# chaitjo/efficient-gnns

Hardware: NVIDIA H100
Metric: edges aggregated/s (fwd+bwd), 3-layer GCN student + logit-KD, ARXIV-shape (higher is better)
Workload: dtype f32

## Files before the change

### efficient-gnns_b200/csrc/gemm_tf32x3.cu

```cuda
#include <cuda.h>

#include "common.cuh"
#include "tc_common.cuh"

namespace b200gnn {
namespace gemm {
using namespace tc;

constexpr int BM = 128, BK = 32;
constexpr int THREADS = 384;
constexpr int CONSUMER_WARPS = 8;
constexpr int TILE_BYTES = BM * BK * 4;
constexpr int BAR_BYTES = 256;
constexpr int EPI_BYTES = CONSUMER_WARPS * 16 * 32 * 4;
constexpr int STAT_MAX_N = 256;
constexpr int STAT_BYTES = CONSUMER_WARPS * 2 * STAT_MAX_N * 4;
constexpr int XY_ROWS = 16;
constexpr int XY_SLOT_BYTES = 2 * XY_ROWS * 32 * 4;
constexpr int XY_BYTES = CONSUMER_WARPS * 2 * XY_SLOT_BYTES;
constexpr int XY_BAR_OFF = 128;
constexpr int BNBWD_TMA_MAX_K = 128;

template <int BN_T, int NSTAGE, int EXTRA = 0>
struct Cfg {
  static constexpr int BN = BN_T, STAGES = NSTAGE;
  static constexpr int B_TILE_BYTES = BN_T * BK * 4;
  static constexpr int STAGE_BYTES = TILE_BYTES + 2 * B_TILE_BYTES;
  static constexpr int ACC = BN_T / 2;
  static constexpr int SMEM_BYTES = NSTAGE * STAGE_BYTES + BAR_BYTES + EPI_BYTES + STAT_BYTES + EXTRA + 1024;
  static_assert(B_TILE_BYTES % 1024 == 0 && (BN_T == 128 || BN_T == 48), "tile shape (wgmma wrappers: N = 128, 48)");
  static_assert(2 * NSTAGE * 8 <= XY_BAR_OFF, "barrier block");
  static_assert(SMEM_BYTES <= 232448, "shared memory");
};

__device__ __forceinline__ void mma(float (&d)[64], const uint32_t (&a)[4], uint64_t b, uint32_t s) { wgmma_tf32_n128_rs(d, a, b, s); }
__device__ __forceinline__ void mma(float (&d)[24], const uint32_t (&a)[4], uint64_t b, uint32_t s) { wgmma_tf32_n48_rs(d, a, b, s); }

__device__ __forceinline__ uint32_t a_frag_offset(int r0, int lane) { return r0 * 128 + ((lane >> 2) << 4) + (lane & 3) * 4; }
__device__ __forceinline__ void load_a(uint32_t frag, uint32_t (&v)[BK / 8][4]) {
  asm("" : "+r"(frag));
#pragma unroll
  for (int k = 0; k < BK / 8; ++k)
#pragma unroll
    for (int i = 0; i < 4; ++i) v[k][i] = lds32((frag ^ ((2 * k + (i >> 1)) << 4)) + (i & 1) * 8 * 128);
}

__device__ __forceinline__ int stg(int r, int c4) { return r * 32 + ((c4 ^ (r & 7)) << 2); }

struct Params {
  float* C;
  const float* bias;
  int64_t ldc;
  int32_t M, N, K;
  int32_t accumulate;
  float* Cp[16];
  int32_t n_peer, kc;
  int64_t row_off;
  int32_t bcast;
  int32_t stat_mode;
  float* stat_partial;
  const float* bn_x;
  const float* bn_y;
  const float* bn_mean;
  const float* bn_invstd;
  float inv_keep;
  const float* act_scale;
  const float* act_shift;
  const uint32_t* act_bits;
  int32_t act_words;
  const float* act_slope;
  double* slope_partial;
  const int64_t* row_idx;
};

template <bool ACT>
__device__ __forceinline__ void load_bn_chunk(const Params& p, int m0, int col, int q, int lane, float4 (&x)[4], float4 (&y)[4]) {
  if (col + 32 > p.N) return;
  const int sub = lane >> 3, cq = (lane & 7) * 4;
#pragma unroll
  for (int it = 0; it < 4; ++it) {
    const int grow = m0 + q * 16 + it * 4 + sub;
    if (grow < p.M) {
      const size_t o = (size_t)grow * p.ldc + col + cq;
      if (!ACT) x[it] = __ldg(reinterpret_cast<const float4*>(p.bn_x + o));
      y[it] = __ldg(reinterpret_cast<const float4*>(p.bn_y + o));
    }
  }
}

__device__ __forceinline__ void load_bits_chunk(const Params& p, int m0, int col, int q, int lane, uint32_t (&w)[4]) {
  const int sub = lane >> 3;
#pragma unroll
  for (int it = 0; it < 4; ++it) {
    const int grow = m0 + q * 16 + it * 4 + sub;
    w[it] = grow < p.M ? __ldg(p.act_bits + (size_t)grow * p.act_words + (col >> 5)) : 0u;
  }
}

__device__ __forceinline__ uint32_t act1(uint32_t y, float sc, float sh, uint32_t keep, float inv_keep) {
  return keep ? __float_as_uint(fmaxf(fmaf(__uint_as_float(y), sc, sh), 0.f) * inv_keep) : 0u;
}

__device__ __forceinline__ uint32_t prelu1(uint32_t z, float slope, uint32_t keep, float inv_keep) {
  const float x = __uint_as_float(z);
  return keep ? __float_as_uint((x > 0.f ? x : slope * x) * inv_keep) : 0u;
}

template <class C, int STAT, bool PEER, bool ACT = false, bool PRELU = false, bool ROWIDX = false>
__global__ void __launch_bounds__(THREADS, 1)
gemm_tf32x3_kernel(const __grid_constant__ CUtensorMap tmA, const __grid_constant__ CUtensorMap tmBhi,
                   const __grid_constant__ CUtensorMap tmBlo, const __grid_constant__ CUtensorMap tmX,
                   const __grid_constant__ CUtensorMap tmY, const Params p) {
  constexpr bool BNB = STAT == 2 || STAT == 3;
  constexpr bool XYTMA = STAT == 3;
  constexpr bool COLSTAT = STAT >= 1 && STAT <= 3;
  constexpr bool PRB = STAT == 4;
  constexpr bool PRO = (ACT || PRELU) && !STAT;
  constexpr int BN = C::BN, STAGES = C::STAGES, STAGE_BYTES = C::STAGE_BYTES, B_TILE_BYTES = C::B_TILE_BYTES, ACC = C::ACC;
  extern __shared__ uint8_t smem_raw[];
  uint8_t* smem = reinterpret_cast<uint8_t*>((reinterpret_cast<uintptr_t>(smem_raw) + 1023) & ~(uintptr_t)1023);
  uint64_t* bars = reinterpret_cast<uint64_t*>(smem + STAGES * STAGE_BYTES);
  uint64_t* full = bars;
  uint64_t* empty = bars + STAGES;
  float* epi_smem = reinterpret_cast<float*>(smem + STAGES * STAGE_BYTES + BAR_BYTES);
  float* stat_smem = reinterpret_cast<float*>(smem + STAGES * STAGE_BYTES + BAR_BYTES + EPI_BYTES);
  uint8_t* xy_smem = smem + STAGES * STAGE_BYTES + BAR_BYTES + EPI_BYTES + STAT_BYTES;
  uint64_t* xy_full = reinterpret_cast<uint64_t*>(smem + STAGES * STAGE_BYTES + XY_BAR_OFF);

  const int warp = threadIdx.x >> 5, lane = threadIdx.x & 31;

  if (threadIdx.x == 0) {
    for (int s = 0; s < STAGES; ++s) { mbar_init(&full[s], 1); mbar_init(&empty[s], 256); }
    if (XYTMA)
      for (int i = 0; i < 2 * CONSUMER_WARPS; ++i) mbar_init(&xy_full[i], 1);
    asm volatile("fence.mbarrier_init.release.cluster;" ::: "memory");
  }
  __syncthreads();

  const int num_m = (p.M + BM - 1) / BM, num_n = (p.N + BN - 1) / BN;
  const int num_tiles = num_m * num_n;
  const int num_kb = (p.K + BK - 1) / BK;

  if (warp < 4) {
    regs_dec<40>();
    if (threadIdx.x == 0) {
      int s = 0; uint32_t ph = 0;
      for (int tile = blockIdx.x; tile < num_tiles; tile += gridDim.x) {
        const int m0 = (tile / num_n) * BM, n0 = (tile % num_n) * BN;
        for (int kb = 0; kb < num_kb; ++kb) {
          mbar_wait(&empty[s], ph ^ 1);
          uint8_t* st = smem + s * STAGE_BYTES;
          mbar_expect_tx(&full[s], TILE_BYTES + 2 * B_TILE_BYTES);
          tma_load_2d(&tmA, &full[s], st, kb * BK, m0);
          tma_load_2d(&tmBhi, &full[s], st + TILE_BYTES, kb * BK, n0);
          tma_load_2d(&tmBlo, &full[s], st + TILE_BYTES + B_TILE_BYTES, kb * BK, n0);
          if (++s == STAGES) { s = 0; ph ^= 1; }
        }
      }
    }
    return;
  }
  regs_inc<232>();

  const int q = warp - 4;
  const bool vec_ok = PEER ? true : ((p.ldc % 4 == 0) && ((reinterpret_cast<uintptr_t>(p.C) & 15) == 0));
  float* stat = stat_smem + q * (2 * STAT_MAX_N);
  if (COLSTAT) {
    for (int i = lane; i < 2 * p.N; i += 32) stat[i] = 0.f;
    __syncwarp();
  }
  constexpr int NCHUNK = (BN + 31) / 32;
  uint8_t* xy = xy_smem + q * (2 * XY_SLOT_BYTES);
  uint64_t* xyb = xy_full + q * 2;
  int n_mine = 0;
  if (XYTMA) {
    for (int tt = blockIdx.x; tt < num_tiles; tt += gridDim.x) n_mine += NCHUNK;
    if (lane == 0)
      for (int g = 0; g < 2 && g < n_mine; ++g) {
        const int tt = blockIdx.x + (g / NCHUNK) * gridDim.x, cc = g % NCHUNK;
        mbar_expect_tx(&xyb[g], ACT ? XY_SLOT_BYTES / 2 : XY_SLOT_BYTES);
        if (!ACT)
          tma_load_2d(&tmX, &xyb[g], xy + g * XY_SLOT_BYTES, (tt % num_n) * BN + cc * 32, (tt / num_n) * BM + q * XY_ROWS);
        tma_load_2d(&tmY, &xyb[g], xy + g * XY_SLOT_BYTES + XY_SLOT_BYTES / 2, (tt % num_n) * BN + cc * 32,
                    (tt / num_n) * BM + q * XY_ROWS);
      }
  }
  const float* act_ss = stat_smem;
  if (ACT && !STAT) {
    for (int c = threadIdx.x - 128; c < num_kb * BK; c += 256) {
      const int w = c & 31;
      const float2 v = c < p.K ? make_float2(__ldg(p.act_scale + c), __ldg(p.act_shift + c)) : make_float2(0.f, 0.f);
      *reinterpret_cast<float2*>(stat_smem + (c >> 5) * 64 + (w & 3) * 16 + (w >> 3) * 4 + ((w >> 2) & 1) * 2) = v;
    }
    named_sync(1, 256);
  }
  const int arow = q * 16 + (lane >> 2);
  auto act_words = [&](int tile, int kb, uint32_t (&w)[2]) {
    const int r = (tile / num_n) * BM + arow;
    w[0] = r < p.M ? __ldg(p.act_bits + (size_t)r * p.act_words + kb) : 0u;
    w[1] = r + 8 < p.M ? __ldg(p.act_bits + (size_t)(r + 8) * p.act_words + kb) : 0u;
  };
  uint32_t wnext[2] = {0u, 0u};
  if (PRO && blockIdx.x < num_tiles) act_words(blockIdx.x, 0, wnext);
  const float slope = (PRELU || PRB) ? __ldg(p.act_slope) : 0.f;
  double sg = 0.0;
  float acc[ACC], sum[ACC];
  uint32_t ah0[BK / 8][4], al0[BK / 8][4], ah1[BK / 8][4], al1[BK / 8][4];
  const uint32_t frag = a_frag_offset(q * 16 + (lane >> 2), lane);
  int s = 0; uint32_t ph = 0;
  int g_chunk = 0;
  for (int tile = blockIdx.x; tile < num_tiles; tile += gridDim.x) {
    const int m0 = (tile / num_n) * BM, n0 = (tile % num_n) * BN;
#pragma unroll
    for (int i = 0; i < ACC; ++i) sum[i] = acc[i] = 0.f;
    int prev = 0;
    auto stage = [&](int kb, uint32_t (&h)[BK / 8][4], uint32_t (&l)[BK / 8][4]) {
      uint32_t wcur[2];
      if (PRO) {
        wcur[0] = wnext[0] >> (lane & 3); wcur[1] = wnext[1] >> (lane & 3);
        if (kb + 1 < num_kb) act_words(tile, kb + 1, wnext);
        else if (tile + (int)gridDim.x < num_tiles) act_words(tile + gridDim.x, 0, wnext);
      }
      mbar_wait(&full[s], ph);
      uint8_t* st = smem + s * STAGE_BYTES;
      load_a(smem_u32(st) + frag, h);
      if (ACT && !STAT) {
        const float4* ss = reinterpret_cast<const float4*>(act_ss + kb * 64 + (lane & 3) * 16);
#pragma unroll
        for (int k = 0; k < BK / 8; ++k) {
          const float4 t = ss[k];
#pragma unroll
          for (int i = 0; i < 4; ++i)
            h[k][i] = act1(h[k][i], (i >> 1) ? t.z : t.x, (i >> 1) ? t.w : t.y, (wcur[i & 1] >> (8 * k + 4 * (i >> 1))) & 1u,
                           p.inv_keep);
        }
      }
      if (PRELU && !STAT) {
#pragma unroll
        for (int k = 0; k < BK / 8; ++k)
#pragma unroll
          for (int i = 0; i < 4; ++i)
            h[k][i] = prelu1(h[k][i], slope, (wcur[i & 1] >> (8 * k + 4 * (i >> 1))) & 1u, p.inv_keep);
      }
#pragma unroll
      for (int k = 0; k < BK / 8; ++k)
#pragma unroll
        for (int i = 0; i < 4; ++i) split1(h[k][i], h[k][i], l[k][i]);
      reg_fence(h); reg_fence(l);
      if (kb > 0) {
        wgmma_wait<0>();
        acc_fence(acc);
#pragma unroll
        for (int i = 0; i < ACC; ++i) sum[i] += acc[i];
        mbar_arrive(&empty[prev]);
      }
      wgmma_fence();
      const uint32_t sb = smem_u32(st + TILE_BYTES);
#pragma unroll
      for (int k = 0; k < BK / 8; ++k) {
        const uint32_t koff = k * 32;
        mma(acc, l[k], make_desc_k128(sb + koff), k != 0);
        mma(acc, h[k], make_desc_k128(sb + B_TILE_BYTES + koff), 1);
      }
#pragma unroll
      for (int k = 0; k < BK / 8; ++k) mma(acc, h[k], make_desc_k128(sb + k * 32), 1);
      wgmma_commit();
      prev = s;
      if (++s == STAGES) { s = 0; ph ^= 1; }
    };
    for (int kb = 0; kb < num_kb; kb += 2) {
      stage(kb, ah0, al0);
      if (kb + 1 < num_kb) stage(kb + 1, ah1, al1);
    }
    wgmma_wait<0>();
    acc_fence(acc);
#pragma unroll
    for (int i = 0; i < ACC; ++i) sum[i] += acc[i];
    mbar_arrive(&empty[prev]);

    float* tile_s = epi_smem + q * (16 * 32);
#pragma unroll
    for (int c = 0; c < NCHUNK; ++c, ++g_chunk) {
      const int col0 = n0 + c * 32;
      float4 xr[4], yr[4];
      if (STAT == 2) load_bn_chunk<ACT>(p, m0, col0, q, lane, xr, yr);
      if (PRB) load_bn_chunk<true>(p, m0, col0, q, lane, xr, yr);
#pragma unroll
      for (int jj = 0; jj < 4; ++jj) {
        const int j = c * 4 + jj;
        if (j * 8 < BN) {
          const int r0 = lane >> 2, cc = jj * 8 + 2 * (lane & 3);
          *reinterpret_cast<float2*>(tile_s + stg(r0, cc >> 2) + (cc & 3)) = make_float2(sum[4 * j], sum[4 * j + 1]);
          *reinterpret_cast<float2*>(tile_s + stg(r0 + 8, cc >> 2) + (cc & 3)) = make_float2(sum[4 * j + 2], sum[4 * j + 3]);
        }
      }
      __syncwarp();
      if (vec_ok && col0 + 32 <= p.N) {
        const float* xs = reinterpret_cast<const float*>(xy + (g_chunk & 1) * XY_SLOT_BYTES);
        const float* ys = xs + XY_ROWS * 32;
        if (XYTMA) mbar_wait(&xyb[g_chunk & 1], (uint32_t)((g_chunk >> 1) & 1));
        const int sub = lane >> 3, cq = (lane & 7) * 4;
        float4 b4 = make_float4(0.f, 0.f, 0.f, 0.f);
        if (p.bias) b4 = make_float4(__ldg(p.bias + col0 + cq), __ldg(p.bias + col0 + cq + 1), __ldg(p.bias + col0 + cq + 2),
                                     __ldg(p.bias + col0 + cq + 3));
        float4 s4 = make_float4(0.f, 0.f, 0.f, 0.f), q4 = s4, mu4 = s4, is4 = s4, sc4 = s4, sh4 = s4;
        if (BNB) {
          mu4 = __ldg(reinterpret_cast<const float4*>(p.bn_mean + col0 + cq));
          is4 = __ldg(reinterpret_cast<const float4*>(p.bn_invstd + col0 + cq));
        }
        uint32_t wb[4];
        if (BNB && ACT) {
          sc4 = __ldg(reinterpret_cast<const float4*>(p.act_scale + col0 + cq));
          sh4 = __ldg(reinterpret_cast<const float4*>(p.act_shift + col0 + cq));
          load_bits_chunk(p, m0, col0, q, lane, wb);
        }
        if (PRB) load_bits_chunk(p, m0, col0, q, lane, wb);
#pragma unroll
        for (int it = 0; it < 4; ++it) {
          const int rr = it * 4 + sub;
          const int grow = m0 + q * 16 + rr;
          float4 v = *reinterpret_cast<const float4*>(tile_s + stg(rr, lane & 7));
          v.x += b4.x; v.y += b4.y; v.z += b4.z; v.w += b4.w;
          if (PEER && grow < p.M && p.bcast) {
            for (int r = 0; r < p.n_peer; ++r)
              *reinterpret_cast<float4*>(p.Cp[r] + (size_t)(p.row_off + grow) * p.ldc + col0 + cq) = v;
          } else if (grow < p.M) {
            float4* dst;
            if (PEER) {
              const int r = col0 / p.kc;
              dst = reinterpret_cast<float4*>(p.Cp[r] + (size_t)(p.row_off + grow) * p.kc + (col0 - r * p.kc) + cq);
            } else {
              const int64_t crow = ROWIDX ? __ldg(p.row_idx + grow) : (int64_t)grow;
              dst = reinterpret_cast<float4*>(p.C + (size_t)crow * p.ldc + col0 + cq);
            }
            if (!PEER && p.accumulate) { const float4 o = *dst; v.x += o.x; v.y += o.y; v.z += o.z; v.w += o.w; }
            if (STAT == 1) {
              vstat(s4, q4, v);
            } else if (BNB) {
              float4 x = make_float4(0.f, 0.f, 0.f, 0.f);
              if (!ACT) x = XYTMA ? *reinterpret_cast<const float4*>(xs + rr * 32 + cq) : xr[it];
              const float4 y = XYTMA ? *reinterpret_cast<const float4*>(ys + rr * 32 + cq) : yr[it];
              if (ACT) {
                const uint32_t b = wb[it] >> cq;
                v.x = (b & 1u) && fmaf(y.x, sc4.x, sh4.x) > 0.f ? v.x * p.inv_keep : 0.f;
                v.y = (b & 2u) && fmaf(y.y, sc4.y, sh4.y) > 0.f ? v.y * p.inv_keep : 0.f;
                v.z = (b & 4u) && fmaf(y.z, sc4.z, sh4.z) > 0.f ? v.z * p.inv_keep : 0.f;
                v.w = (b & 8u) && fmaf(y.w, sc4.w, sh4.w) > 0.f ? v.w * p.inv_keep : 0.f;
              } else {
                v.x = x.x > 0.f ? v.x * p.inv_keep : 0.f; v.y = x.y > 0.f ? v.y * p.inv_keep : 0.f;
                v.z = x.z > 0.f ? v.z * p.inv_keep : 0.f; v.w = x.w > 0.f ? v.w * p.inv_keep : 0.f;
              }
              s4.x += v.x; s4.y += v.y; s4.z += v.z; s4.w += v.w;
              q4.x = fmaf(v.x, (y.x - mu4.x) * is4.x, q4.x); q4.y = fmaf(v.y, (y.y - mu4.y) * is4.y, q4.y);
              q4.z = fmaf(v.z, (y.z - mu4.z) * is4.z, q4.z); q4.w = fmaf(v.w, (y.w - mu4.w) * is4.w, q4.w);
            } else if (PRB) {
              const float4 z = yr[it];
              const uint32_t b = wb[it] >> cq;
              const float gx = (b & 1u) ? v.x * p.inv_keep : 0.f, gy = (b & 2u) ? v.y * p.inv_keep : 0.f;
              const float gz = (b & 4u) ? v.z * p.inv_keep : 0.f, gw = (b & 8u) ? v.w * p.inv_keep : 0.f;
              if (!(z.x > 0.f)) sg += (double)(gx * z.x);
              if (!(z.y > 0.f)) sg += (double)(gy * z.y);
              if (!(z.z > 0.f)) sg += (double)(gz * z.z);
              if (!(z.w > 0.f)) sg += (double)(gw * z.w);
              v.x = z.x > 0.f ? gx : gx * slope; v.y = z.y > 0.f ? gy : gy * slope;
              v.z = z.z > 0.f ? gz : gz * slope; v.w = z.w > 0.f ? gw : gw * slope;
            }
            *dst = v;
          }
        }
        if (COLSTAT) {
#pragma unroll
          for (int d = 8; d <= 16; d <<= 1) {
            s4.x += __shfl_xor_sync(0xffffffffu, s4.x, d); s4.y += __shfl_xor_sync(0xffffffffu, s4.y, d);
            s4.z += __shfl_xor_sync(0xffffffffu, s4.z, d); s4.w += __shfl_xor_sync(0xffffffffu, s4.w, d);
            q4.x += __shfl_xor_sync(0xffffffffu, q4.x, d); q4.y += __shfl_xor_sync(0xffffffffu, q4.y, d);
            q4.z += __shfl_xor_sync(0xffffffffu, q4.z, d); q4.w += __shfl_xor_sync(0xffffffffu, q4.w, d);
          }
          if (lane < 8) {
            float4* ps = reinterpret_cast<float4*>(stat + col0 + cq);
            float4* pq = reinterpret_cast<float4*>(stat + p.N + col0 + cq);
            float4 a0 = *ps, a1 = *pq;
            a0.x += s4.x; a0.y += s4.y; a0.z += s4.z; a0.w += s4.w;
            a1.x += q4.x; a1.y += q4.y; a1.z += q4.z; a1.w += q4.w;
            *ps = a0; *pq = a1;
          }
        }
        __syncwarp();
        if (XYTMA && lane == 0 && g_chunk + 2 < n_mine) {
          const int g = g_chunk + 2, tt = blockIdx.x + (g / NCHUNK) * gridDim.x, cc = g % NCHUNK;
          uint8_t* dst = xy + (g & 1) * XY_SLOT_BYTES;
          mbar_expect_tx(&xyb[g & 1], ACT ? XY_SLOT_BYTES / 2 : XY_SLOT_BYTES);
          if (!ACT) tma_load_2d(&tmX, &xyb[g & 1], dst, (tt % num_n) * BN + cc * 32, (tt / num_n) * BM + q * XY_ROWS);
          tma_load_2d(&tmY, &xyb[g & 1], dst + XY_SLOT_BYTES / 2, (tt % num_n) * BN + cc * 32, (tt / num_n) * BM + q * XY_ROWS);
        }
      } else {
        const int rr = lane & 15, cb = (lane >> 4) * 16, grow = m0 + q * 16 + rr;
        if (grow < p.M && col0 + cb < p.N) {
          for (int jx = 0; jx < 16; ++jx) {
            const int cc = cb + jx, col = col0 + cc;
            if (col >= p.N) break;
            const float v = tile_s[stg(rr, cc >> 2) + (cc & 3)] + (p.bias ? __ldg(p.bias + col) : 0.f);
            if (PEER && p.bcast) {
              for (int r = 0; r < p.n_peer; ++r) p.Cp[r][(size_t)(p.row_off + grow) * p.ldc + col] = v;
            } else if (!PEER) {
              float* dst = p.C + (size_t)(ROWIDX ? __ldg(p.row_idx + grow) : (int64_t)grow) * p.ldc + col;
              *dst = v + (p.accumulate ? *dst : 0.f);
            }
          }
        }
        __syncwarp();
      }
    }
  }
  if (COLSTAT) {
    __syncwarp();
    float* out = p.stat_partial + (size_t)(blockIdx.x * CONSUMER_WARPS + q) * 2 * p.N;
    for (int i = lane; i < 2 * p.N; i += 32) out[i] = stat[i];
  }
  if (PRB) {
#pragma unroll
    for (int d = 16; d > 0; d >>= 1) sg += __shfl_xor_sync(0xffffffffu, sg, d);
    if (lane == 0) p.slope_partial[blockIdx.x * CONSUMER_WARPS + q] = sg;
  }
}

__global__ void __launch_bounds__(32) slope_grad_finalize_kernel(const double* __restrict__ part, int n, float* __restrict__ out,
                                                                 int accumulate) {
  double a = 0.0;
  for (int i = threadIdx.x; i < n; i += 32) a += part[i];
#pragma unroll
  for (int d = 16; d > 0; d >>= 1) a += __shfl_xor_sync(0xffffffffu, a, d);
  if (threadIdx.x == 0) out[0] = accumulate ? out[0] + (float)a : (float)a;
}

__global__ void __launch_bounds__(256) split_tf32_kernel(const float* __restrict__ W, int64_t rows, int64_t cols,
                                                         int transpose, float* __restrict__ hi, float* __restrict__ lo) {
  const int64_t n = rows * cols;
  for (int64_t i = (int64_t)blockIdx.x * blockDim.x + threadIdx.x; i < n; i += (int64_t)gridDim.x * blockDim.x) {
    const int64_t r = i / cols, c = i - r * cols;
    uint32_t h, l;
    split1(__float_as_uint(W[i]), h, l);
    const int64_t o = transpose ? c * rows + r : i;
    hi[o] = __uint_as_float(h);
    lo[o] = __uint_as_float(l);
  }
}

static bool make_map(CUtensorMap* m, const float* base, int64_t rows, int64_t cols, int64_t ld, int box_rows, bool swizzle = true) {
  EncodeTiledFn fn = encode_fn();
  if (!fn) return false;
  cuuint64_t dims[2] = {(cuuint64_t)cols, (cuuint64_t)rows};
  cuuint64_t strides[1] = {(cuuint64_t)ld * 4};
  cuuint32_t box[2] = {(cuuint32_t)BK, (cuuint32_t)box_rows};
  cuuint32_t estr[2] = {1, 1};
  return fn(m, CU_TENSOR_MAP_DATA_TYPE_FLOAT32, 2, const_cast<float*>(base), dims, strides, box, estr,
            CU_TENSOR_MAP_INTERLEAVE_NONE, swizzle ? CU_TENSOR_MAP_SWIZZLE_128B : CU_TENSOR_MAP_SWIZZLE_NONE,
            CU_TENSOR_MAP_L2_PROMOTION_L2_256B, CU_TENSOR_MAP_FLOAT_OOB_FILL_NONE) == CUDA_SUCCESS;
}

template <class C, int STAT = 0, bool PEER = false, bool ACT = false, bool PRELU = false, bool ROWIDX = false>
static int launch(const float* A, int64_t lda, const float* B_hi, const float* B_lo, int64_t ldb, const Params& p,
                  cudaStream_t stream) {
  CUtensorMap tA, tBh, tBl, tX, tY;
  if (!make_map(&tA, A, p.M, p.K, lda, BM) || !make_map(&tBh, B_hi, p.N, p.K, ldb, C::BN) ||
      !make_map(&tBl, B_lo, p.N, p.K, ldb, C::BN))
    return B200GNN_ERR_UNSUPPORTED;
  tX = tA; tY = tA;
  if (STAT == 3 && ((!ACT && !make_map(&tX, p.bn_x, p.M, p.N, p.ldc, XY_ROWS, false)) ||
                    !make_map(&tY, p.bn_y, p.M, p.N, p.ldc, XY_ROWS, false)))
    return B200GNN_ERR_UNSUPPORTED;
  int dev = 0, sms = 132;
  cudaGetDevice(&dev);
  static bool attr_set[64] = {};
  if (dev >= 0 && dev < 64 && !attr_set[dev]) {
    cudaError_t e = cudaFuncSetAttribute(gemm_tf32x3_kernel<C, STAT, PEER, ACT, PRELU, ROWIDX>, cudaFuncAttributeMaxDynamicSharedMemorySize,
                                         C::SMEM_BYTES);
    if (e != cudaSuccess) { set_cuda_error(e); return B200GNN_ERR_CUDA; }
    attr_set[dev] = true;
  }
  const int tiles = ((p.M + BM - 1) / BM) * ((p.N + C::BN - 1) / C::BN);
  cudaDeviceGetAttribute(&sms, cudaDevAttrMultiProcessorCount, dev);
  const int grid = tiles < sms ? tiles : sms;
  gemm_tf32x3_kernel<C, STAT, PEER, ACT, PRELU, ROWIDX><<<grid, THREADS, C::SMEM_BYTES, stream>>>(tA, tBh, tBl, tX, tY, p);
  return check_launch();
}

}
}

using namespace b200gnn;

extern "C" int b200gnn_split_tf32_f32(const float* W, int64_t rows, int64_t cols, int transpose, float* hi, float* lo,
                                      void* stream) {
  if (!W || !hi || !lo || rows <= 0 || cols <= 0) return B200GNN_ERR_BAD_ARG;
  const int64_t n = rows * cols;
  int grid = (int)((n + 255) / 256);
  if (grid > 132 * 8) grid = 132 * 8;
  gemm::split_tf32_kernel<<<grid, 256, 0, (cudaStream_t)stream>>>(W, rows, cols, transpose, hi, lo);
  return check_launch();
}

static int g_bnbwd_variant = 0;
extern "C" void b200gnn_gemm_set_bnbwd_variant(int v) { g_bnbwd_variant = v; }

static int gemm_dispatch(const float* A, int64_t lda, const float* B_hi, const float* B_lo, int64_t ldb, float* C, int64_t ldc,
                         int64_t M, int64_t N, int64_t K, const float* bias, int accumulate, void* stream,
                         const gemm::Params* st = nullptr, const gemm::Params* act = nullptr,
                         const gemm::Params* prelu = nullptr) {
  if (!A || !B_hi || !B_lo || !C || M <= 0 || N <= 0 || K <= 0 || lda < K || ldb < K || ldc < N ||
      M >= INT32_MAX || N >= INT32_MAX || K >= INT32_MAX)
    return B200GNN_ERR_BAD_ARG;
  if (lda % 4 || ldb % 4 || !aligned_to(A, 16) || !aligned_to(B_hi, 16) || !aligned_to(B_lo, 16))
    return B200GNN_ERR_UNSUPPORTED;
  gemm::Params p{};
  p.C = C; p.bias = bias; p.ldc = ldc; p.M = (int32_t)M; p.N = (int32_t)N; p.K = (int32_t)K; p.accumulate = accumulate ? 1 : 0;
  p.n_peer = 0; p.kc = 0; p.row_off = 0; p.bcast = 0;
  if (act) {
    if (!act->act_scale || !act->act_shift || !act->act_bits || !aligned_to(act->act_scale, 16) || !aligned_to(act->act_shift, 16))
      return B200GNN_ERR_BAD_ARG;
    p.act_scale = act->act_scale; p.act_shift = act->act_shift; p.act_bits = act->act_bits; p.act_words = act->act_words;
    p.inv_keep = act->inv_keep;
  }
  if (prelu) {
    if (!prelu->act_slope || !prelu->act_bits) return B200GNN_ERR_BAD_ARG;
    p.act_slope = prelu->act_slope; p.act_bits = prelu->act_bits; p.act_words = prelu->act_words; p.inv_keep = prelu->inv_keep;
    if (prelu->stat_mode == 0) {
      if (N <= 48) return gemm::launch<gemm::Cfg<48, 6>, 0, false, false, true>(A, lda, B_hi, B_lo, ldb, p, (cudaStream_t)stream);
      return gemm::launch<gemm::Cfg<128, 4>, 0, false, false, true>(A, lda, B_hi, B_lo, ldb, p, (cudaStream_t)stream);
    }
    if (N % 32 || ldc % 4 || !aligned_to(C, 16) || !prelu->bn_y || !aligned_to(prelu->bn_y, 16) || !prelu->slope_partial)
      return B200GNN_ERR_UNSUPPORTED;
    p.stat_mode = 4; p.bn_y = prelu->bn_y; p.slope_partial = prelu->slope_partial;
    return gemm::launch<gemm::Cfg<128, 4>, 4>(A, lda, B_hi, B_lo, ldb, p, (cudaStream_t)stream);
  }
  if (act && !st) {
    if (K > (int64_t)gemm::STAT_BYTES / 8) return B200GNN_ERR_UNSUPPORTED;
    if (N <= 48) return gemm::launch<gemm::Cfg<48, 6>, 0, false, true>(A, lda, B_hi, B_lo, ldb, p, (cudaStream_t)stream);
    return gemm::launch<gemm::Cfg<128, 4>, 0, false, true>(A, lda, B_hi, B_lo, ldb, p, (cudaStream_t)stream);
  }
  if (st) {
    if (N % 32 || N > gemm::STAT_MAX_N || N <= 48 || ldc % 4 || !aligned_to(C, 16) || !st->stat_partial) return B200GNN_ERR_UNSUPPORTED;
    p.stat_mode = st->stat_mode; p.stat_partial = st->stat_partial; p.bn_x = st->bn_x; p.bn_y = st->bn_y;
    p.bn_mean = st->bn_mean; p.bn_invstd = st->bn_invstd; p.inv_keep = st->inv_keep;
    if (p.stat_mode == 1) return gemm::launch<gemm::Cfg<128, 4>, 1>(A, lda, B_hi, B_lo, ldb, p, (cudaStream_t)stream);
    const bool tma = N % 128 == 0 && (g_bnbwd_variant == 1 || (g_bnbwd_variant == 0 && K < gemm::BNBWD_TMA_MAX_K));
    if (act)
      return tma ? gemm::launch<gemm::Cfg<128, 2, gemm::XY_BYTES>, 3, false, true>(A, lda, B_hi, B_lo, ldb, p, (cudaStream_t)stream)
                 : gemm::launch<gemm::Cfg<128, 4>, 2, false, true>(A, lda, B_hi, B_lo, ldb, p, (cudaStream_t)stream);
    if (tma) return gemm::launch<gemm::Cfg<128, 2, gemm::XY_BYTES>, 3>(A, lda, B_hi, B_lo, ldb, p, (cudaStream_t)stream);
    return gemm::launch<gemm::Cfg<128, 4>, 2>(A, lda, B_hi, B_lo, ldb, p, (cudaStream_t)stream);
  }
  if (N <= 48) return gemm::launch<gemm::Cfg<48, 6>>(A, lda, B_hi, B_lo, ldb, p, (cudaStream_t)stream);
  return gemm::launch<gemm::Cfg<128, 4>>(A, lda, B_hi, B_lo, ldb, p, (cudaStream_t)stream);
}

extern "C" int64_t b200gnn_gemm_stat_slots(int64_t M, int64_t N) {
  if (M <= 0 || N <= 0) return B200GNN_ERR_BAD_ARG;
  int dev = 0, sms = 132;
  cudaGetDevice(&dev);
  cudaDeviceGetAttribute(&sms, cudaDevAttrMultiProcessorCount, dev);
  const int64_t tiles = ((M + gemm::BM - 1) / gemm::BM) * ((N + 127) / 128);
  return gemm::CONSUMER_WARPS * (tiles < sms ? tiles : sms);
}

extern "C" int b200gnn_gemm_tf32x3_stats_f32(const float* A, int64_t lda, const float* B_hi, const float* B_lo, int64_t ldb,
                                             float* C, int64_t ldc, int64_t M, int64_t N, int64_t K, const float* bias,
                                             int accumulate, float* partial, int64_t slots, void* stream) {
  if (!partial || slots < b200gnn_gemm_stat_slots(M, N) || (accumulate && bias)) return B200GNN_ERR_BAD_ARG;
  gemm::Params st{};
  st.stat_mode = 1; st.stat_partial = partial;
  return gemm_dispatch(A, lda, B_hi, B_lo, ldb, C, ldc, M, N, K, bias, accumulate, stream, &st);
}

extern "C" int b200gnn_gemm_tf32x3_bnbwd_f32(const float* A, int64_t lda, const float* B_hi, const float* B_lo, int64_t ldb,
                                             float* C, int64_t ldc, int64_t M, int64_t N, int64_t K, int accumulate,
                                             const float* Xout, const float* Y, const float* mean, const float* invstd, float p_drop,
                                             float* partial, int64_t slots, void* stream) {
  if (!partial || !Xout || !Y || !mean || !invstd || p_drop < 0.f || p_drop >= 1.f || slots < b200gnn_gemm_stat_slots(M, N))
    return B200GNN_ERR_BAD_ARG;
  if (!aligned_to(Xout, 16) || !aligned_to(Y, 16) || !aligned_to(mean, 16) || !aligned_to(invstd, 16)) return B200GNN_ERR_UNSUPPORTED;
  gemm::Params st{};
  st.stat_mode = 2; st.stat_partial = partial; st.bn_x = Xout; st.bn_y = Y; st.bn_mean = mean; st.bn_invstd = invstd;
  st.inv_keep = p_drop > 0.f ? 1.f / (1.f - p_drop) : 1.f;
  return gemm_dispatch(A, lda, B_hi, B_lo, ldb, C, ldc, M, N, K, nullptr, accumulate, stream, &st);
}

extern "C" int b200gnn_gemm_tf32x3_bnbwd_bits_f32(const float* A, int64_t lda, const float* B_hi, const float* B_lo, int64_t ldb,
                                                  float* C, int64_t ldc, int64_t M, int64_t N, int64_t K, int accumulate,
                                                  const uint32_t* bits, const float* Y, const float* mean, const float* invstd,
                                                  const float* scale, const float* shift, float p_drop, float* partial,
                                                  int64_t slots, void* stream) {
  if (!partial || !bits || !Y || !mean || !invstd || p_drop < 0.f || p_drop >= 1.f || slots < b200gnn_gemm_stat_slots(M, N))
    return B200GNN_ERR_BAD_ARG;
  if (!aligned_to(Y, 16) || !aligned_to(mean, 16) || !aligned_to(invstd, 16)) return B200GNN_ERR_UNSUPPORTED;
  gemm::Params st{}, act{};
  st.stat_mode = 2; st.stat_partial = partial; st.bn_y = Y; st.bn_mean = mean; st.bn_invstd = invstd;
  st.inv_keep = p_drop > 0.f ? 1.f / (1.f - p_drop) : 1.f;
  act.act_scale = scale; act.act_shift = shift; act.act_bits = bits; act.act_words = (int32_t)((N + 31) / 32);
  act.inv_keep = st.inv_keep;
  return gemm_dispatch(A, lda, B_hi, B_lo, ldb, C, ldc, M, N, K, nullptr, accumulate, stream, &st, &act);
}

extern "C" int b200gnn_gemm_tf32x3_act_f32(const float* Y, int64_t lda, const float* B_hi, const float* B_lo, int64_t ldb,
                                           float* C, int64_t ldc, int64_t M, int64_t N, int64_t K, const float* bias,
                                           const float* scale, const float* shift, const uint32_t* bits, float p_drop,
                                           void* stream) {
  if (p_drop < 0.f || p_drop >= 1.f) return B200GNN_ERR_BAD_ARG;
  gemm::Params act{};
  act.act_scale = scale; act.act_shift = shift; act.act_bits = bits; act.act_words = (int32_t)((K + 31) / 32);
  act.inv_keep = p_drop > 0.f ? 1.f / (1.f - p_drop) : 1.f;
  return gemm_dispatch(Y, lda, B_hi, B_lo, ldb, C, ldc, M, N, K, bias, 0, stream, nullptr, &act);
}

extern "C" int b200gnn_gemm_tf32x3_prelu_f32(const float* Z, int64_t lda, const float* B_hi, const float* B_lo, int64_t ldb,
                                             float* C, int64_t ldc, int64_t M, int64_t N, int64_t K, const float* bias,
                                             const float* slope, const uint32_t* bits, float p_drop, void* stream) {
  if (p_drop < 0.f || p_drop >= 1.f) return B200GNN_ERR_BAD_ARG;
  gemm::Params pr{};
  pr.stat_mode = 0; pr.act_slope = slope; pr.act_bits = bits; pr.act_words = (int32_t)((K + 31) / 32);
  pr.inv_keep = p_drop > 0.f ? 1.f / (1.f - p_drop) : 1.f;
  return gemm_dispatch(Z, lda, B_hi, B_lo, ldb, C, ldc, M, N, K, bias, 0, stream, nullptr, nullptr, &pr);
}

extern "C" int b200gnn_gemm_tf32x3_prelu_bwd_f32(const float* A, int64_t lda, const float* B_hi, const float* B_lo, int64_t ldb,
                                                 float* C, int64_t ldc, int64_t M, int64_t N, int64_t K, int accumulate,
                                                 const float* Z, const uint32_t* bits, const float* slope, float p_drop,
                                                 float* slope_grad, int slope_accumulate, double* partial, int64_t slots,
                                                 void* stream) {
  if (!Z || !slope_grad || !partial || p_drop < 0.f || p_drop >= 1.f || M <= 0 || N <= 0) return B200GNN_ERR_BAD_ARG;
  const int64_t used = b200gnn_gemm_stat_slots(M, N);
  if (slots < used) return B200GNN_ERR_BAD_ARG;
  gemm::Params pr{};
  pr.stat_mode = 4; pr.act_slope = slope; pr.act_bits = bits; pr.act_words = (int32_t)((N + 31) / 32);
  pr.inv_keep = p_drop > 0.f ? 1.f / (1.f - p_drop) : 1.f;
  pr.bn_y = Z; pr.slope_partial = partial;
  int rc = gemm_dispatch(A, lda, B_hi, B_lo, ldb, C, ldc, M, N, K, nullptr, accumulate, stream, nullptr, nullptr, &pr);
  if (rc) return rc;
  gemm::slope_grad_finalize_kernel<<<1, 32, 0, (cudaStream_t)stream>>>(partial, (int)used, slope_grad, slope_accumulate ? 1 : 0);
  return check_launch();
}

extern "C" int b200gnn_gemm_tf32x3_f32(const float* A, int64_t lda, const float* B_hi, const float* B_lo, int64_t ldb,
                                       float* C, int64_t ldc, int64_t M, int64_t N, int64_t K, const float* bias,
                                       void* stream) {
  return gemm_dispatch(A, lda, B_hi, B_lo, ldb, C, ldc, M, N, K, bias, 0, stream);
}

extern "C" int b200gnn_gemm_tf32x3_acc_f32(const float* A, int64_t lda, const float* B_hi, const float* B_lo, int64_t ldb,
                                           float* C, int64_t ldc, int64_t M, int64_t N, int64_t K, void* stream) {
  return gemm_dispatch(A, lda, B_hi, B_lo, ldb, C, ldc, M, N, K, nullptr, 1, stream);
}

extern "C" int b200gnn_gemm_tf32x3_rowidx_f32(const float* A, int64_t lda, const float* B_hi, const float* B_lo, int64_t ldb,
                                              float* C, int64_t ldc, int64_t M, int64_t N, int64_t K, const int64_t* row_idx,
                                              void* stream) {
  if (!A || !B_hi || !B_lo || !C || !row_idx || M <= 0 || N <= 0 || K <= 0 || lda < K || ldb < K || ldc < N ||
      M >= INT32_MAX || N >= INT32_MAX || K >= INT32_MAX)
    return B200GNN_ERR_BAD_ARG;
  if (lda % 4 || ldb % 4 || !aligned_to(A, 16) || !aligned_to(B_hi, 16) || !aligned_to(B_lo, 16)) return B200GNN_ERR_UNSUPPORTED;
  gemm::Params p{};
  p.C = C; p.bias = nullptr; p.ldc = ldc; p.M = (int32_t)M; p.N = (int32_t)N; p.K = (int32_t)K; p.accumulate = 0;
  p.row_idx = row_idx;
  if (N <= 48) return gemm::launch<gemm::Cfg<48, 6>, 0, false, false, false, true>(A, lda, B_hi, B_lo, ldb, p, (cudaStream_t)stream);
  return gemm::launch<gemm::Cfg<128, 4>, 0, false, false, false, true>(A, lda, B_hi, B_lo, ldb, p, (cudaStream_t)stream);
}

extern "C" int b200gnn_gemm_tf32x3_scatter_f32(const float* A, int64_t lda, const float* B_hi, const float* B_lo, int64_t ldb,
                                               float* const* C_ptrs, int32_t world, int64_t row_off, int64_t M, int64_t N, int64_t K,
                                               const float* bias, void* stream) {
  if (!A || !B_hi || !B_lo || !C_ptrs || world <= 0 || world > 16 || M <= 0 || N <= 0 || K <= 0 || lda < K || ldb < K || row_off < 0 ||
      M >= INT32_MAX || N >= INT32_MAX || K >= INT32_MAX)
    return B200GNN_ERR_BAD_ARG;
  if (N % world || (N / world) % 32 || N <= 48) return B200GNN_ERR_UNSUPPORTED;
  if (lda % 4 || ldb % 4 || !aligned_to(A, 16) || !aligned_to(B_hi, 16) || !aligned_to(B_lo, 16)) return B200GNN_ERR_UNSUPPORTED;
  gemm::Params p{};
  p.C = nullptr; p.bias = bias; p.ldc = N; p.M = (int32_t)M; p.N = (int32_t)N; p.K = (int32_t)K; p.accumulate = 0;
  p.n_peer = world; p.kc = (int32_t)(N / world); p.row_off = row_off; p.bcast = 0;
  for (int q = 0; q < world; ++q) {
    if (!C_ptrs[q] || !aligned_to(C_ptrs[q], 16)) return B200GNN_ERR_BAD_ARG;
    p.Cp[q] = C_ptrs[q];
  }
  return gemm::launch<gemm::Cfg<128, 4>, 0, true>(A, lda, B_hi, B_lo, ldb, p, (cudaStream_t)stream);
}

extern "C" int b200gnn_gemm_tf32x3_bcast_f32(const float* A, int64_t lda, const float* B_hi, const float* B_lo, int64_t ldb,
                                             float* const* C_ptrs, int32_t world, int64_t row_off, int64_t ldc, int64_t M, int64_t N,
                                             int64_t K, const float* bias, void* stream) {
  if (!A || !B_hi || !B_lo || !C_ptrs || world <= 0 || world > 16 || M <= 0 || N <= 0 || K <= 0 || lda < K || ldb < K || ldc < N ||
      row_off < 0 || M >= INT32_MAX || N >= INT32_MAX || K >= INT32_MAX)
    return B200GNN_ERR_BAD_ARG;
  if (lda % 4 || ldb % 4 || ldc % 4 || !aligned_to(A, 16) || !aligned_to(B_hi, 16) || !aligned_to(B_lo, 16)) return B200GNN_ERR_UNSUPPORTED;
  gemm::Params p{};
  p.C = C_ptrs[0]; p.bias = bias; p.ldc = ldc; p.M = (int32_t)M; p.N = (int32_t)N; p.K = (int32_t)K; p.accumulate = 0;
  p.n_peer = world; p.kc = (int32_t)N; p.row_off = row_off; p.bcast = 1;
  for (int q = 0; q < world; ++q) {
    if (!C_ptrs[q] || !aligned_to(C_ptrs[q], 16)) return B200GNN_ERR_BAD_ARG;
    p.Cp[q] = C_ptrs[q];
  }
  if (N <= 48) return gemm::launch<gemm::Cfg<48, 6>, 0, true>(A, lda, B_hi, B_lo, ldb, p, (cudaStream_t)stream);
  return gemm::launch<gemm::Cfg<128, 4>, 0, true>(A, lda, B_hi, B_lo, ldb, p, (cudaStream_t)stream);
}
```

Before: 3.949 billion.

## Prefetch Y-only TMA slots deeper and hoist keep-bit loads per tile in BN-backward GEMM

For the BN-backward GEMM with a fused activation, the kernel now always takes the TMA epilogue path. It stages only Y, not X, in a configurable number of per-warp slots (three here), and uses three main-loop stages instead of two or four. The keep-bit dropout mask words are loaded once per tile ahead of time and passed between lanes with shuffles, instead of a global load per chunk. The aim is to hide epilogue global-memory latency, at the cost of reshaping the shared-memory and barrier layout, and K-block pipeline depth differs from the previous variants.

```diff
diff --git a/efficient-gnns_b200/csrc/gemm_tf32x3.cu b/efficient-gnns_b200/csrc/gemm_tf32x3.cu
--- a/efficient-gnns_b200/csrc/gemm_tf32x3.cu
+++ b/efficient-gnns_b200/csrc/gemm_tf32x3.cu
@@ -18,18 +18,22 @@
 constexpr int XY_ROWS = 16;
 constexpr int XY_SLOT_BYTES = 2 * XY_ROWS * 32 * 4;
 constexpr int XY_BYTES = CONSUMER_WARPS * 2 * XY_SLOT_BYTES;
+constexpr int Y_SLOT_BYTES = XY_ROWS * 32 * 4;
 constexpr int XY_BAR_OFF = 128;
 constexpr int BNBWD_TMA_MAX_K = 128;
 
-template <int BN_T, int NSTAGE, int EXTRA = 0>
+template <int BN_T, int NSTAGE, int EXTRA = 0, int YD = 0>
 struct Cfg {
-  static constexpr int BN = BN_T, STAGES = NSTAGE;
+  static constexpr int BN = BN_T, STAGES = NSTAGE, YDEPTH = YD;
   static constexpr int B_TILE_BYTES = BN_T * BK * 4;
   static constexpr int STAGE_BYTES = TILE_BYTES + 2 * B_TILE_BYTES;
   static constexpr int ACC = BN_T / 2;
-  static constexpr int SMEM_BYTES = NSTAGE * STAGE_BYTES + BAR_BYTES + EPI_BYTES + STAT_BYTES + EXTRA + 1024;
+  static constexpr int BAR = YD > 2 ? 384 : BAR_BYTES;
+  static constexpr int SMEM_BYTES =
+      NSTAGE * STAGE_BYTES + BAR + EPI_BYTES + STAT_BYTES + EXTRA + YD * CONSUMER_WARPS * Y_SLOT_BYTES + 1024;
   static_assert(B_TILE_BYTES % 1024 == 0 && (BN_T == 128 || BN_T == 48), "tile shape (wgmma wrappers: N = 128, 48)");
-  static_assert(2 * NSTAGE * 8 <= XY_BAR_OFF, "barrier block");
+  static_assert(2 * NSTAGE * 8 <= XY_BAR_OFF && XY_BAR_OFF + CONSUMER_WARPS * (YD > 2 ? YD : 2) * 8 <= BAR, "barrier block");
+  static_assert(YD <= 4 && BAR % 128 == 0, "Y slots: 128-byte aligned TMA destinations");
   static_assert(SMEM_BYTES <= 232448, "shared memory");
 };
 
@@ -116,23 +120,28 @@
   constexpr bool COLSTAT = STAT >= 1 && STAT <= 3;
   constexpr bool PRB = STAT == 4;
   constexpr bool PRO = (ACT || PRELU) && !STAT;
+  constexpr bool TILE_BITS = BNB && ACT;
+  static_assert(!TILE_BITS || XYTMA, "the keep-bit mask reads Y from the TMA slots");
   constexpr int BN = C::BN, STAGES = C::STAGES, STAGE_BYTES = C::STAGE_BYTES, B_TILE_BYTES = C::B_TILE_BYTES, ACC = C::ACC;
   extern __shared__ uint8_t smem_raw[];
   uint8_t* smem = reinterpret_cast<uint8_t*>((reinterpret_cast<uintptr_t>(smem_raw) + 1023) & ~(uintptr_t)1023);
   uint64_t* bars = reinterpret_cast<uint64_t*>(smem + STAGES * STAGE_BYTES);
   uint64_t* full = bars;
   uint64_t* empty = bars + STAGES;
-  float* epi_smem = reinterpret_cast<float*>(smem + STAGES * STAGE_BYTES + BAR_BYTES);
-  float* stat_smem = reinterpret_cast<float*>(smem + STAGES * STAGE_BYTES + BAR_BYTES + EPI_BYTES);
-  uint8_t* xy_smem = smem + STAGES * STAGE_BYTES + BAR_BYTES + EPI_BYTES + STAT_BYTES;
+  float* epi_smem = reinterpret_cast<float*>(smem + STAGES * STAGE_BYTES + C::BAR);
+  float* stat_smem = reinterpret_cast<float*>(smem + STAGES * STAGE_BYTES + C::BAR + EPI_BYTES);
+  uint8_t* xy_smem = smem + STAGES * STAGE_BYTES + C::BAR + EPI_BYTES + STAT_BYTES;
   uint64_t* xy_full = reinterpret_cast<uint64_t*>(smem + STAGES * STAGE_BYTES + XY_BAR_OFF);
+  constexpr int NSLOT = ACT ? C::YDEPTH : 2;
+  constexpr int SLOT_BYTES = ACT ? Y_SLOT_BYTES : XY_SLOT_BYTES, Y_OFF = ACT ? 0 : XY_SLOT_BYTES / 2;
+  static_assert(!XYTMA || (ACT ? NSLOT >= 1 : C::YDEPTH == 0), "XYTMA slots");
 
   const int warp = threadIdx.x >> 5, lane = threadIdx.x & 31;
 
   if (threadIdx.x == 0) {
     for (int s = 0; s < STAGES; ++s) { mbar_init(&full[s], 1); mbar_init(&empty[s], 256); }
     if (XYTMA)
-      for (int i = 0; i < 2 * CONSUMER_WARPS; ++i) mbar_init(&xy_full[i], 1);
+      for (int i = 0; i < NSLOT * CONSUMER_WARPS; ++i) mbar_init(&xy_full[i], 1);
     asm volatile("fence.mbarrier_init.release.cluster;" ::: "memory");
   }
   __syncthreads();
@@ -170,21 +179,21 @@
     __syncwarp();
   }
   constexpr int NCHUNK = (BN + 31) / 32;
-  uint8_t* xy = xy_smem + q * (2 * XY_SLOT_BYTES);
-  uint64_t* xyb = xy_full + q * 2;
-  int n_mine = 0;
-  if (XYTMA) {
-    for (int tt = blockIdx.x; tt < num_tiles; tt += gridDim.x) n_mine += NCHUNK;
-    if (lane == 0)
-      for (int g = 0; g < 2 && g < n_mine; ++g) {
-        const int tt = blockIdx.x + (g / NCHUNK) * gridDim.x, cc = g % NCHUNK;
-        mbar_expect_tx(&xyb[g], ACT ? XY_SLOT_BYTES / 2 : XY_SLOT_BYTES);
-        if (!ACT)
-          tma_load_2d(&tmX, &xyb[g], xy + g * XY_SLOT_BYTES, (tt % num_n) * BN + cc * 32, (tt / num_n) * BM + q * XY_ROWS);
-        tma_load_2d(&tmY, &xyb[g], xy + g * XY_SLOT_BYTES + XY_SLOT_BYTES / 2, (tt % num_n) * BN + cc * 32,
-                    (tt / num_n) * BM + q * XY_ROWS);
-      }
-  }
+  uint8_t* xy = xy_smem + q * (NSLOT * SLOT_BYTES);
+  uint64_t* xyb = xy_full + q * NSLOT;
+  int xt = blockIdx.x, xc = 0;
+  auto request = [&](int slot) {
+    if (xt >= num_tiles) return;
+    const int c0 = (xt % num_n) * BN + xc * 32, r0 = (xt / num_n) * BM + q * XY_ROWS;
+    if (lane == 0) {
+      mbar_expect_tx(&xyb[slot], ACT ? Y_SLOT_BYTES : XY_SLOT_BYTES);
+      if (!ACT) tma_load_2d(&tmX, &xyb[slot], xy + slot * SLOT_BYTES, c0, r0);
+      tma_load_2d(&tmY, &xyb[slot], xy + slot * SLOT_BYTES + Y_OFF, c0, r0);
+    }
+    if (++xc == NCHUNK || c0 + 32 >= p.N) { xc = 0; xt += gridDim.x; }
+  };
+  if (XYTMA)
+    for (int i = 0; i < NSLOT; ++i) request(i);
   const float* act_ss = stat_smem;
   if (ACT && !STAT) {
     for (int c = threadIdx.x - 128; c < num_kb * BK; c += 256) {
@@ -202,13 +211,20 @@
   };
   uint32_t wnext[2] = {0u, 0u};
   if (PRO && blockIdx.x < num_tiles) act_words(blockIdx.x, 0, wnext);
+  auto tile_words = [&](int tile, uint32_t (&w)[2]) {
+    const int wd = ((tile % num_n) * BN >> 5) + (lane & 3);
+    w[0] = w[1] = 0u;
+    if (tile < num_tiles && wd < p.act_words) act_words(tile, wd, w);
+  };
+  uint32_t bw[2];
+  if (TILE_BITS) tile_words(blockIdx.x, bw);
   const float slope = (PRELU || PRB) ? __ldg(p.act_slope) : 0.f;
   double sg = 0.0;
   float acc[ACC], sum[ACC];
   uint32_t ah0[BK / 8][4], al0[BK / 8][4], ah1[BK / 8][4], al1[BK / 8][4];
   const uint32_t frag = a_frag_offset(q * 16 + (lane >> 2), lane);
   int s = 0; uint32_t ph = 0;
-  int g_chunk = 0;
+  int xslot = 0; uint32_t xph = 0;
   for (int tile = blockIdx.x; tile < num_tiles; tile += gridDim.x) {
     const int m0 = (tile / num_n) * BM, n0 = (tile % num_n) * BN;
 #pragma unroll
@@ -280,7 +296,7 @@
 
     float* tile_s = epi_smem + q * (16 * 32);
 #pragma unroll
-    for (int c = 0; c < NCHUNK; ++c, ++g_chunk) {
+    for (int c = 0; c < NCHUNK; ++c) {
       const int col0 = n0 + c * 32;
       float4 xr[4], yr[4];
       if (STAT == 2) load_bn_chunk<ACT>(p, m0, col0, q, lane, xr, yr);
@@ -296,9 +312,9 @@
       }
       __syncwarp();
       if (vec_ok && col0 + 32 <= p.N) {
-        const float* xs = reinterpret_cast<const float*>(xy + (g_chunk & 1) * XY_SLOT_BYTES);
-        const float* ys = xs + XY_ROWS * 32;
-        if (XYTMA) mbar_wait(&xyb[g_chunk & 1], (uint32_t)((g_chunk >> 1) & 1));
+        const float* xs = reinterpret_cast<const float*>(xy + xslot * SLOT_BYTES);
+        const float* ys = reinterpret_cast<const float*>(xy + xslot * SLOT_BYTES + Y_OFF);
+        if (XYTMA) mbar_wait(&xyb[xslot], xph);
         const int sub = lane >> 3, cq = (lane & 7) * 4;
         float4 b4 = make_float4(0.f, 0.f, 0.f, 0.f);
         if (p.bias) b4 = make_float4(__ldg(p.bias + col0 + cq), __ldg(p.bias + col0 + cq + 1), __ldg(p.bias + col0 + cq + 2),
@@ -309,10 +325,11 @@
           is4 = __ldg(reinterpret_cast<const float4*>(p.bn_invstd + col0 + cq));
         }
         uint32_t wb[4];
-        if (BNB && ACT) {
+        if (TILE_BITS) {
           sc4 = __ldg(reinterpret_cast<const float4*>(p.act_scale + col0 + cq));
           sh4 = __ldg(reinterpret_cast<const float4*>(p.act_shift + col0 + cq));
-          load_bits_chunk(p, m0, col0, q, lane, wb);
+#pragma unroll
+          for (int it = 0; it < 4; ++it) wb[it] = __shfl_sync(0xffffffffu, bw[it >> 1], ((it & 1) * 4 + sub) * 4 + c);
         }
         if (PRB) load_bits_chunk(p, m0, col0, q, lane, wb);
 #pragma unroll
@@ -386,12 +403,9 @@
           }
         }
         __syncwarp();
-        if (XYTMA && lane == 0 && g_chunk + 2 < n_mine) {
-          const int g = g_chunk + 2, tt = blockIdx.x + (g / NCHUNK) * gridDim.x, cc = g % NCHUNK;
-          uint8_t* dst = xy + (g & 1) * XY_SLOT_BYTES;
-          mbar_expect_tx(&xyb[g & 1], ACT ? XY_SLOT_BYTES / 2 : XY_SLOT_BYTES);
-          if (!ACT) tma_load_2d(&tmX, &xyb[g & 1], dst, (tt % num_n) * BN + cc * 32, (tt / num_n) * BM + q * XY_ROWS);
-          tma_load_2d(&tmY, &xyb[g & 1], dst + XY_SLOT_BYTES / 2, (tt % num_n) * BN + cc * 32, (tt / num_n) * BM + q * XY_ROWS);
+        if (XYTMA) {
+          request(xslot);
+          if (++xslot == NSLOT) { xslot = 0; xph ^= 1; }
         }
       } else {
         const int rr = lane & 15, cb = (lane >> 4) * 16, grow = m0 + q * 16 + rr;
@@ -411,6 +425,7 @@
         __syncwarp();
       }
     }
+    if (TILE_BITS) tile_words(tile + gridDim.x, bw);
   }
   if (COLSTAT) {
     __syncwarp();
@@ -543,10 +558,8 @@
     p.stat_mode = st->stat_mode; p.stat_partial = st->stat_partial; p.bn_x = st->bn_x; p.bn_y = st->bn_y;
     p.bn_mean = st->bn_mean; p.bn_invstd = st->bn_invstd; p.inv_keep = st->inv_keep;
     if (p.stat_mode == 1) return gemm::launch<gemm::Cfg<128, 4>, 1>(A, lda, B_hi, B_lo, ldb, p, (cudaStream_t)stream);
+    if (act) return gemm::launch<gemm::Cfg<128, 3, 0, 3>, 3, false, true>(A, lda, B_hi, B_lo, ldb, p, (cudaStream_t)stream);
     const bool tma = N % 128 == 0 && (g_bnbwd_variant == 1 || (g_bnbwd_variant == 0 && K < gemm::BNBWD_TMA_MAX_K));
-    if (act)
-      return tma ? gemm::launch<gemm::Cfg<128, 2, gemm::XY_BYTES>, 3, false, true>(A, lda, B_hi, B_lo, ldb, p, (cudaStream_t)stream)
-                 : gemm::launch<gemm::Cfg<128, 4>, 2, false, true>(A, lda, B_hi, B_lo, ldb, p, (cudaStream_t)stream);
     if (tma) return gemm::launch<gemm::Cfg<128, 2, gemm::XY_BYTES>, 3>(A, lda, B_hi, B_lo, ldb, p, (cudaStream_t)stream);
     return gemm::launch<gemm::Cfg<128, 4>, 2>(A, lda, B_hi, B_lo, ldb, p, (cudaStream_t)stream);
   }
```

After: 3.988 billion, median of 6. About the same (+1.0%).
